# jvmncs/safe-grid-agents

Measured on AMD Instinct MI355X. Metric: env-steps/sec at 1M concurrent BoatRace envs, higher is better.
Workload: dtype int8

## Files before the change

safe-grid-agents_amd/csrc/sgk_api.hip:

```cpp
#include <hip/hip_runtime.h>

#include <algorithm>
#include <cmath>
#include <cstdio>
#include <cstdlib>
#include <cstring>
#include <memory>
#include <utility>

#include "sgk_host_core.h"
#include "sgk_kernels.h"

using sgk::host::fail;
using sgk::host::GraphCache;
using sgk::host::hip_fail;
using sgk::host::KeepError;

namespace {

__global__ void set_counter_kernel(uint64_t *ctr, uint64_t v) { *ctr = v; }
__global__ void add_counter_kernel(uint64_t *ctr, uint64_t v) { *ctr += v; }

}

// ... 174 lines not shown
  *out = nullptr;
  if (n_envs <= 0 || n_envs > ((int64_t)1 << 31) - 512) return fail(SGK_ERR_INVALID, "n_envs out of range");
  const bool host_visible = (layout & SGK_MEM_HOST_VISIBLE) != 0;
  layout &= ~SGK_MEM_HOST_VISIBLE;
  if (layout != SGK_LAYOUT_PITCHED && layout != SGK_LAYOUT_COMPACT) return fail(SGK_ERR_INVALID, "unknown layout");
  if (host_visible && n_envs > 65536) return fail(SGK_ERR_INVALID, "SGK_MEM_HOST_VISIBLE is for small batches (<= 65536 envs)");
  int n_dev = 0;
  hipError_t e = hipGetDeviceCount(&n_dev);
  if (e != hipSuccess || n_dev <= 0)
    return fail(SGK_ERR_NODEVICE, "libsgk has no CPU fallback and found no HIP device%s%s", e != hipSuccess ? ": " : "",
                e != hipSuccess ? hipGetErrorString(e) : "");
  if (device < 0 || device >= n_dev) return fail(SGK_ERR_INVALID, "device ordinal out of range");
  sgk_env *h = sgk::host::host_new<sgk_env>();
  sgk::Shard &s = h->sh;
  if (sgk_build_rules(env_id, &s.rules_host) != 0) {
    delete h;
    return fail(SGK_ERR_INVALID, "unknown env_id");
  }
  s.env_id = env_id;
  s.device = device;
  s.n = n_envs;
  s.seed = seed;
  s.env_base = env_index_base;
  s.n_cells = s.rules_host.n_cells;
  s.n_states = s.rules_host.n_states;
  const int pitched = ((s.n_cells + 15) / 16) * 16;
  s.layout = layout;
  s.pitch = (s.layout == SGK_LAYOUT_COMPACT) ? s.n_cells : pitched;
  const char *ng = getenv("SGK_NO_GRAPH");
  h->use_graph = !(ng && ng[0] == '1');

#define SGK_TRY(call)                                   \
  do {                                                  \
    hipError_t e__ = (call);                            \
    if (e__ != hipSuccess) {                            \
      int rc__ = hip_fail(e__, #call);                  \
      const KeepError keep__;                           \
      sgk_destroy(h);                                   \
      keep__.restore();                                 \
      return rc__;                                      \
    }                                                   \
  } while (0)

  SGK_TRY(hipSetDevice(device));
  hipDeviceProp_t prop;
  SGK_TRY(hipGetDeviceProperties(&prop, device));
  s.n_cus = prop.multiProcessorCount > 0 ? prop.multiProcessorCount : 256;
  s.max_grid = s.n_cus * 6;
  if (const char *mg = getenv("SGK_MAX_GRID")) {
    int v = atoi(mg);
    if (v >= 64) s.max_grid = v;
  }
  s.stream_grid = s.n_cus * 16;
  if (const char *nt = getenv("SGK_RING_NT")) s.ring_nt_mode = nt[0] == '0' ? 0 : (nt[0] == '1' ? 1 : -1);
  if (const char *sg = getenv("SGK_STREAM_GRID")) {
    int v = atoi(sg);
    if (v >= 64) s.stream_grid = v;
  }
  s.rollout_grid = s.n_cus * 12;
  SGK_TRY(pooled_stream(device, &h->own_stream));
  h->stream = h->own_stream;
  const int64_t n_pad = ((s.n + 255) / 256) * 256;
  const int64_t n_wg = n_pad / 256;
  SGK_TRY(hipMalloc((void **)&s.rules_dev, sgk::SGK_RULES_DEV_BYTES));
  h->host_visible = host_visible;
  if (host_visible) {
    SGK_TRY(hipHostMalloc((void **)&s.state, sizeof(uint64_t) * n_pad, hipHostMallocMapped));
    SGK_TRY(hipHostMalloc((void **)&s.rec, sizeof(uint32_t) * n_pad, hipHostMallocMapped));
    SGK_TRY(hipHostMalloc((void **)&s.boards, (size_t)s.pitch * n_pad, hipHostMallocMapped));
    SGK_TRY(hipHostMalloc((void **)&h->hv_actions, (size_t)n_pad, hipHostMallocMapped));
    const char *srv = getenv("SGK_STEP_SERVER");
    if (n_envs <= 64 && !(srv && srv[0] == '0')) {
      SGK_TRY(hipHostMalloc((void **)&h->srv.mb, sizeof(sgk::SgkMailbox), hipHostMallocMapped));
      memset((void *)h->srv.mb, 0, sizeof(sgk::SgkMailbox));
    }
  } else {
    SGK_TRY(hipMalloc(&s.state, sizeof(uint64_t) * n_pad));
    SGK_TRY(hipMalloc(&s.rec, sizeof(uint32_t) * n_pad));
    SGK_TRY(hipMalloc(&s.boards, (size_t)s.pitch * n_pad));
  }
  if (host_visible) {
    SGK_TRY(hipHostMalloc((void **)&s.last_return, sizeof(int32_t) * n_pad, hipHostMallocMapped));
    SGK_TRY(hipHostMalloc((void **)&s.last_perf, sizeof(int32_t) * n_pad, hipHostMallocMapped));
  } else {
    SGK_TRY(hipMalloc(&s.last_return, sizeof(int32_t) * n_pad));
    SGK_TRY(hipMalloc(&s.last_perf, sizeof(int32_t) * n_pad));
  }
  SGK_TRY(hipMalloc(&s.n_episodes, sizeof(int32_t) * n_pad));
  SGK_TRY(hipMalloc(&s.n_resets, sizeof(int32_t) * n_pad));
  if (env_id == SGK_FRIEND_FOE) SGK_TRY(hipMalloc(&s.aux, sizeof(double) * SGK_AUX_DOUBLES * n_pad));
  SGK_TRY(hipMalloc(&s.metrics, sizeof(int64_t) * SGK_METRICS_LEN));
  SGK_TRY(hipMalloc(&s.metric_slab, sizeof(int64_t) * SGK_METRICS_LEN * SGK_METRIC_SLOTS));
  SGK_TRY(hipMalloc(&s.wg_count, sizeof(int32_t) * n_wg));
  SGK_TRY(hipMalloc(&s.wg_offset, sizeof(int64_t) * n_wg));
  SGK_TRY(hipMalloc(&s.finished_total, sizeof(int64_t)));
  SGK_TRY(hipMalloc(&h->t_dev, sizeof(uint64_t)));
  SGK_TRY(hipHostMalloc((void **)&h->metrics_pinned, sizeof(long long) * SGK_METRICS_LEN, hipHostMallocMapped));
  {
    static_assert(sgk::SGK_RULES_DEV_BYTES <= 8192, "staged on the stack");
    uint8_t image[sgk::SGK_RULES_DEV_BYTES];
    memset(image, 0, sizeof(image));
    memcpy(image, &s.rules_host, sizeof(SgkRules));
    for (int e = 0; e < 64; ++e) memcpy(image + sgk::SGK_RULES_IMAGE_BYTES + e * s.n_cells, s.rules_host.templ, (size_t)s.n_cells);
    SGK_TRY(hipMemcpyAsync(s.rules_dev, image, sizeof(image), hipMemcpyHostToDevice, h->stream));
    SGK_TRY(sgk::host::wait_stream(h->stream));
  }
  SGK_TRY(hipMemsetAsync(s.rec, 0, sizeof(uint32_t) * n_pad, h->stream));
// ... 1263 lines not shown
```

safe-grid-agents_amd/csrc/sgk_host_core.h:

```cpp
#pragma once
#include <hip/hip_runtime.h>
#include <stdarg.h>
#include <stdint.h>
#include <stdio.h>
#include <string.h>

#include <atomic>
#include <map>
#include <memory>
#include <mutex>
#include <new>
#include <utility>
#include <vector>

#include "../../include/sgk.h"
#include "sgk_mailbox.h"

namespace sgk {
namespace host {

constexpr size_t ERROR_BYTES = 640;
inline char *error_buffer() {
  static thread_local char buf[ERROR_BYTES] = "";
  return buf;
}
__attribute__((format(printf, 2, 3))) inline int fail(int code, const char *fmt, ...) {
  char tmp[ERROR_BYTES];
  va_list ap;
  va_start(ap, fmt);
  vsnprintf(tmp, sizeof(tmp), fmt, ap);
  va_end(ap);
  memcpy(error_buffer(), tmp, sizeof(tmp));
  return code;
}
inline int hip_fail(hipError_t e, const char *what) { return fail(SGK_ERR_HIP, "%s: %s", what, hipGetErrorString(e)); }
struct KeepError {
  char saved[ERROR_BYTES];
  KeepError() { memcpy(saved, error_buffer(), ERROR_BYTES); }
  void restore() const { memcpy(error_buffer(), saved, ERROR_BYTES); }
};

#define SGK_HIP(call)                                               \
  do {                                                              \
    hipError_t e__ = (call);                                        \
    if (e__ != hipSuccess) return ::sgk::host::hip_fail(e__, #call); \
  } while (0)

#define SGK_CATCH_STATUS                                                                                        \
  catch (const std::bad_alloc &) { return ::sgk::host::fail(SGK_ERR_NOMEM, "out of host memory"); }           \
  catch (const std::exception &e__) { return ::sgk::host::fail(SGK_ERR_INTERNAL, "internal error: %s", e__.what()); } \
  catch (...) { return ::sgk::host::fail(SGK_ERR_INTERNAL, "internal error (unknown exception)"); }
#define SGK_CATCH_VALUE(v) \
  catch (...) { return (v); }

inline std::atomic<int> &alloc_countdown() {
  static std::atomic<int> c{0};
  return c;
}
inline void alloc_gate() {
  std::atomic<int> &c = alloc_countdown();
  if (c.load(std::memory_order_relaxed) > 0 && c.fetch_sub(1, std::memory_order_relaxed) == 1) throw std::bad_alloc();
}
template <class T>
struct HostAlloc {
  using value_type = T;
  HostAlloc() = default;
  template <class U>
  HostAlloc(const HostAlloc<U> &) {}
  T *allocate(size_t n) {
    alloc_gate();
    return std::allocator<T>().allocate(n);
  }
  void deallocate(T *p, size_t n) { std::allocator<T>().deallocate(p, n); }
  template <class U>
  bool operator==(const HostAlloc<U> &) const { return true; }
  template <class U>
  bool operator!=(const HostAlloc<U> &) const { return false; }
};
template <class T>
using Vec = std::vector<T, HostAlloc<T>>;
template <class K, class V>
using Map = std::map<K, V, std::less<K>, HostAlloc<std::pair<const K, V>>>;
template <class T>
T *host_new() {
  alloc_gate();
  return new T();
}
// ... 379 lines not shown
```

safe-grid-agents_amd/csrc/sgk_kernels.h:

```cpp
#pragma once
#include <hip/hip_runtime.h>
#include <stdint.h>

#include "../../include/sgk.h"
#include "sgk_mailbox.h"
#include "sgk_rules.h"

#define SGK_METRIC_SLOTS 2048

namespace sgk {

constexpr int SGK_RULES_IMAGE_BYTES = 2048;
constexpr int SGK_RULES_DEV_BYTES = SGK_RULES_IMAGE_BYTES + 64 * SGK_CELLS;

struct Shard {
  int env_id = 0, layout = 0, device = 0;
  int n_cells = 0, pitch = 0, n_states = 0;
  int n_cus = 256, max_grid = 2048, stream_grid = 2048, rollout_grid = 2048;
  int ring_nt_mode = -1;
  int64_t n = 0;
  uint64_t seed = 0, env_base = 0, lockstep_t = 0;
  SgkRules rules_host;
  SgkRules *rules_dev = nullptr;
  uint64_t *state = nullptr;
  uint32_t *rec = nullptr;
  int8_t *boards = nullptr;
  int32_t *last_return = nullptr;
  int32_t *last_perf = nullptr;
  int32_t *n_episodes = nullptr;
  int32_t *n_resets = nullptr;
  double *aux = nullptr;
  int64_t *metrics = nullptr;
  int64_t *metric_slab = nullptr;
  int32_t *wg_count = nullptr;
  int64_t *wg_offset = nullptr;
  int64_t *finished_total = nullptr;
};

struct TabqShard {
  double *table = nullptr;
  uint64_t *tags = nullptr;
  double *row_cache = nullptr;
  uint32_t *keys = nullptr;
  int32_t hash_cap = 0;
  int32_t *hash_overflow = nullptr;
  int32_t n_states = 0;
  double lr = 0, discount = 0, eps0 = 0;
  int64_t anneal = 0;
  int64_t t_agent = 0;
  const long long *t_ptr = nullptr;
};

hipError_t launch_step(const Shard &sh, const uint8_t *actions, uint32_t flags, hipStream_t st);
hipError_t launch_env_server(const Shard &sh, const uint8_t *actions, SgkMailbox *mb, uint32_t last, hipStream_t st);
hipError_t launch_rollout_random(const Shard &sh, int32_t n_steps, uint32_t flags, hipStream_t st);
hipError_t launch_rollout_stream(const Shard &sh, int32_t n_steps, uint32_t flags, int8_t *boards_ring, uint32_t *recs_ring,
                                 int32_t ring, int32_t slice0, hipStream_t st);
hipError_t launch_reset(const Shard &sh, const uint8_t *mask, int mode, hipStream_t st);
hipError_t launch_ring_probe(const Shard &sh, int8_t *boards_ring, uint32_t *recs_ring, int32_t ring, uint32_t flags, hipStream_t st);
hipError_t launch_metrics_init(const Shard &sh, hipStream_t st);
hipError_t launch_aux_init(const Shard &sh, hipStream_t st);
hipError_t launch_metrics_reduce(const Shard &sh, hipStream_t st, long long *out_host = nullptr);
hipError_t launch_obs_f32(const Shard &sh, float *dst, hipStream_t st);
struct PolicyWeights {
  const float *w1t, *b1, *w2, *b2, *w3t, *b3;
  int n_hidden;
};
hipError_t launch_policy_act(const Shard &sh, int mode, const PolicyWeights &w, uint8_t *actions, float *scores, double eps,
                             uint64_t draw, const double *eps_dev, const uint64_t *draw_dev, hipStream_t st);
hipError_t launch_policy_rollout(const Shard &sh, int mode, const PolicyWeights &w, double eps, uint64_t draw0, int32_t n_steps,
                                 uint32_t flags, int8_t *states_out, uint8_t *actions_out, uint32_t *recs_out, hipStream_t st);
hipError_t launch_eps_greedy(const Shard &sh, int mode, const float *scores, uint8_t *actions, double eps, uint64_t draw,
// ... 109 lines not shown
```

safe-grid-agents_amd/csrc/sgk_step.hip:

```cpp
#include <type_traits>

#include "sgk_device.h"
#include "sgk_step_store.h"

namespace sgk {

constexpr int STREAM_MIN_WAVES = 4;
#define SGK_TILE_DECLARE(ENV, NC, ON)                                                 \
  __shared__ __attribute__((aligned(16))) uint8_t tile_images[WG / 64][64 * (NC)];    \
  WaveTileLds<ENV, NC> W;                                                             \
  W.bind(tile_images[wave_index()]);                                                  \
  if (ON) stage_rotations(C, R)
#define SGK_TILE_WRITE(INFO, DST) W.write(C, R, (INFO), (DST))

__global__ __launch_bounds__(1024) void metrics_reduce_kernel(const long long *__restrict__ slab, long long *__restrict__ out,
                                                              long long *__restrict__ out_host) {
  __shared__ long long part[1024];
  const int col = threadIdx.x & 15, lane_slot = threadIdx.x >> 4;
  const bool is_max = col >= SGK_M_MAX_RETURN && col <= SGK_M_MAX_MARGIN_POS;
  long long acc = is_max ? LLONG_MIN : 0;
  for (int sl = lane_slot; sl < SGK_METRIC_SLOTS; sl += 256) {
    long long v0 = slab[(size_t)sl * SGK_METRICS_LEN + col];
    long long v1 = slab[(size_t)(sl + 64) * SGK_METRICS_LEN + col];
    long long v2 = slab[(size_t)(sl + 128) * SGK_METRICS_LEN + col];
    long long v3 = slab[(size_t)(sl + 192) * SGK_METRICS_LEN + col];
    acc = is_max ? max(max(acc, v0), max(max(v1, v2), v3)) : acc + ((v0 + v1) + (v2 + v3));
  }
  part[threadIdx.x] = acc;
  __syncthreads();
  for (int half = 32; half >= 1; half >>= 1) {
    if (lane_slot < half) {
      long long o = part[(lane_slot + half) * 16 + col];
      part[threadIdx.x] = is_max ? max(part[threadIdx.x], o) : part[threadIdx.x] + o;
    }
    __syncthreads();
  }
  if (threadIdx.x < 16) {
    out[threadIdx.x] = part[threadIdx.x];
    if (out_host) out_host[threadIdx.x] = part[threadIdx.x];
  }
}

__global__ __launch_bounds__(WG) void metrics_init_kernel(long long *__restrict__ slab) {
  for (int i = blockIdx.x * WG + threadIdx.x; i < SGK_METRIC_SLOTS * SGK_METRICS_LEN; i += gridDim.x * WG) {
    int col = i & 15;
    slab[i] = (col >= SGK_M_MAX_RETURN && col <= SGK_M_MAX_MARGIN_POS) ? LLONG_MIN : 0;
  }
}

constexpr int64_t STEP_SMALL_MAX_ENVS = 65536;

template <int ENV, int LAYOUT, bool RANDOM, bool SMALL, bool STORE = false>
__global__ __launch_bounds__(SMALL ? 64 : WG) void step_kernel(StepArgs a, StepStore st) {
  constexpr int WGT = SMALL ? 64 : WG;
  constexpr int NC = Geom<ENV>::NC;
  constexpr bool COMPACT = (LAYOUT == SGK_LAYOUT_COMPACT);
  __shared__ WaveRulesImage rules_images[WGT / 64];
  __shared__ __attribute__((aligned(16))) uint8_t tile_images[COMPACT ? WGT / 64 : 1][COMPACT ? 64 * NC : 16];
  __shared__ int episode_words[WGT / 64][16];
  const int lane = threadIdx.x & 63, wave = wave_index();
  const int64_t n_wt = (a.n + 63) / 64;
  const int64_t wt0 = (int64_t)blockIdx.x * (WGT / 64) + wave, wstride = (int64_t)gridDim.x * (WGT / 64);
  const bool boards_on = !(a.flags & SGK_F_NO_BOARDS);
  keep_in_sgprs(a.rec, a.boards, a.last_return, a.last_perf);
  keep_in_sgprs(a.n_episodes, a.n_resets, a.metrics, a.aux);
  keep_in_sgprs(a.seed, a.env_base, a.t, a.flags);
// ... 124 lines not shown
    if (req == SGK_SERVER_STOP) break;
    idle_since = 0;
    const uint32_t flags = hi & 0xffu;
    int action = (int)((hi >> 8) & 3u);
    if (a.n > 1) {
      __builtin_amdgcn_fence(__ATOMIC_ACQUIRE, "");
      if (valid) action = (int)(__hip_atomic_load(&a.actions[env], __ATOMIC_RELAXED, __HIP_MEMORY_SCOPE_SYSTEM) & 3u);
    }
    if (flags & SGK_SRV_RESET) {
      if (valid) {
        const int epi = s.epi + 1;
        bump_reset_count<ENV>(a.n_resets, env);
        s = initial_state(R);
        s.epi = epi;
        begin_episode<ENV>(R, s, a.seed, a.env_base + (uint64_t)env, aux_of<ENV>(a.aux, env));
        a.state[env] = pack_state(s);
      }
    } else {
      StepArgs b = a;
      b.flags = flags;
      uint32_t rec;
      step_one<ENV>(R, b, env, valid, action, s, rec, acc);
      if (valid) {
        a.state[env] = pack_state(s);
        a.rec[env] = rec;
      }
    }
    if (!(flags & SGK_F_NO_BOARDS)) {
      if (COMPACT) {
        W.draw_all(C, R, sprite_info<ENV>(R, s));
        W.flush_prefix(a.boards, (int)a.n * NC);
      } else if (valid) {
        write_board_pitched<ENV, Geom<ENV>::PITCH>(R, a.boards, env, s);
      }
    }
    __builtin_amdgcn_fence(__ATOMIC_RELEASE, "");
    asm volatile("s_waitcnt vmcnt(0)" ::: "memory");
    if (lane == 0) __hip_atomic_store(&mb->done, req, __ATOMIC_RELAXED, __HIP_MEMORY_SCOPE_SYSTEM);
    last = req;
  }
  acc_flush(acc, a.metrics);
  __builtin_amdgcn_fence(__ATOMIC_RELEASE, "");
  asm volatile("s_waitcnt vmcnt(0)" ::: "memory");
  if (lane == 0) __hip_atomic_store(&mb->exited, last + 1u, __ATOMIC_RELAXED, __HIP_MEMORY_SCOPE_SYSTEM);
}

hipError_t launch_env_server(const Shard &sh, const uint8_t *actions, SgkMailbox *mb, uint32_t last, hipStream_t st) {
  (void)hipGetLastError();
  StepArgs a = make_step_args(sh, actions, 0);
  SGK_DISPATCH_ENV_LAYOUT(sh.env_id, sh.layout, env_server_kernel<E, L><<<dim3(1), dim3(64), 0, st>>>(a, mb, last));
  return hipGetLastError();
}

struct StreamOut {
  int8_t *boards;
  uint32_t *recs;
  int32_t ring, slice0;
  int32_t tiles_ok;
  int32_t tile_major;
  int32_t ring_nt;
};

template <int ENV, int LAYOUT, bool STREAM>
__global__ __launch_bounds__(WG, STREAM ? STREAM_MIN_WAVES : 1) void rollout_random_kernel(StepArgs a, int32_t n_steps, StreamOut o) {
  constexpr int NC = Geom<ENV>::NC;
  constexpr bool COMPACT = (LAYOUT == SGK_LAYOUT_COMPACT);
  __shared__ SgkRules R;
  __shared__ CompactLds<NC> C;
  uint64_t first_word = 0;
  {
    const int64_t env0 = ((int64_t)blockIdx.x * (WG / 64) + (threadIdx.x >> 6)) * 64 + (threadIdx.x & 63);
    if (STREAM && env0 < a.n) first_word = a.state[env0];
  }
  stage_rules(R, a.rules);
  SGK_TILE_DECLARE(ENV, NC, (COMPACT || STREAM));
  const int lane = threadIdx.x & 63, wave = STREAM ? wave_index() : (int)(threadIdx.x >> 6);
  const bool boards_on = !(a.flags & SGK_F_NO_BOARDS);
  const int64_t n_wt = (a.n + 63) / 64;
  EpisodeAcc acc;
  acc_init(acc);
  for (int64_t wt = (int64_t)blockIdx.x * (WG / 64) + wave; wt < n_wt; wt += (int64_t)gridDim.x * (WG / 64)) {
    const int64_t env = wt * 64 + lane;
    const bool valid = env < a.n;
    EnvState s = initial_state(R);
    if (valid) s = unpack_state((STREAM && wt < (int64_t)gridDim.x * (WG / 64)) ? first_word : a.state[env]);
    load_episode_index<ENV>(s, a.n_resets, env, valid);
    const uint64_t ge = a.env_base + (uint64_t)env;
    AuxRegs ax;
    ax.init();
    if (HasAux<ENV>::value && valid) ax.load(a.aux + env * SGK_AUX_DOUBLES);
    uint32_t x[4] = {0, 0, 0, 0};
    uint32_t rec = 0;
    uint32_t w = 0;
    int last_obs = 0, last_hid = 0, last_done = 0, last_action = 0;
    const bool auto_reset = (a.flags & SGK_F_AUTO_RESET) != 0;
    const bool whole_tile = wt * 64 + 64 <= a.n;
    int32_t slice = o.slice0;
    uint32_t drawn = sprite_info<ENV>(R, s);
    if (STREAM && boards_on) W.draw_all(C, R, drawn);
    if (STREAM) {
    const bool tm = o.boards && o.tile_major;
    const bool tiles = o.boards ? (tm || (o.tiles_ok && whole_tile)) : COMPACT;
    const bool flush_nt = o.boards && o.ring_nt;
    uint32_t *recs_p = !o.recs ? a.rec + env
                               : (o.tile_major ? o.recs + (wt * (int64_t)o.ring + slice) * 64 + lane : o.recs + (int64_t)slice * a.n + env);
    const int64_t rec_stride = !o.recs ? 0 : (o.tile_major ? 64 : a.n);
    int8_t *dense = !o.boards ? a.boards
                              : (tm ? o.boards + ((wt * (int64_t)o.ring + slice) - wt) * 64 * NC : o.boards + (int64_t)slice * a.n * NC);
    const int64_t brd_stride = !o.boards ? 0 : (tm ? (int64_t)64 * NC : a.n * (int64_t)NC);
    const int64_t rec_wrap = rec_stride * (o.ring - 1), brd_wrap = brd_stride * (o.ring - 1);
    uint32_t left = 0;
#pragma nounroll
    for (int32_t k = 0; k < n_steps; ++k) {
      if (left == 0) {
        const uint64_t t = a.t + (uint64_t)k;
        const uint32_t tl = (uint32_t)t;
        if (k == 0 || (tl & 63u) == 0)
          philox4x32_10((uint32_t)ge, (uint32_t)(ge >> 32), (uint32_t)(t >> 6), 0u, (uint32_t)a.seed, (uint32_t)(a.seed >> 32), x);
        const uint32_t j = (tl >> 4) & 3u;
        w = (j == 0 ? x[0] : (j == 1 ? x[1] : (j == 2 ? x[2] : x[3]))) >> (2 * (tl & 15u));
        left = 16 - (tl & 15u);
      }
      --left;
      int action = (int)(w & 3u);
      w >>= 2;
      const bool live = valid && !s.over;
      if (live) action = env_actual_action<ENV>(R, s, a.seed, ge, action);
      last_action = action;
      last_obs = 0;
      last_hid = 0;
      last_done = valid ? 1 : 0;
      if (live) {
        int r_obs, r_hid, term;
        if (HasAux<ENV>::value) transition_with<ENV>(R, s, action, r_obs, r_hid, term, ax);
        else transition<ENV>(R, s, action, r_obs, r_hid, term);
        s.frame += 1;
        s.ret += r_obs;
        s.hid += r_hid;
        last_obs = r_obs;
        last_hid = r_hid;
        last_done = 0;
        if (term || s.frame >= R.max_iterations) {
          last_done = 1;
          acc_add(acc, true, s.ret, s.hid);
          int64_t env_here = env;
          asm volatile("" : "+v"(env_here));
          a.last_return[env_here] = s.ret;
          a.last_perf[env_here] = s.hid;
          bump_episode_count(a.n_episodes, env_here);
          if (auto_reset) {
            const int epi = s.epi + 1;
            s = initial_state(R);
            s.epi = epi;
            if (HasAux<ENV>::value) begin_episode_with<ENV>(R, s, a.seed, ge, ax);
            else begin_episode<ENV>(R, s, a.seed, ge);
          } else {
            s.over = 1;
          }
        }
      }
      const uint32_t rk = pack_rec(last_obs, last_hid, last_done, last_action);
      if (valid) *recs_p = rk;
      if (boards_on) {
        const uint32_t now = sprite_info<ENV>(R, s);
        W.update(R, drawn, now);
        drawn = now;
        if (tiles) {
          if (flush_nt) W.template flush<RING_STORE_AUX>(dense + wt * 64 * NC);
          else W.flush(dense + wt * 64 * NC);
        }
        else if (o.boards) { if (valid) write_row_bytes<ENV, NC>(R, dense + env * NC, s); }
        else if (valid) write_board_pitched<ENV, Geom<ENV>::PITCH>(R, a.boards, env, s);
      }
      if (++slice == o.ring) {
        slice = 0;
        recs_p -= rec_wrap;
        dense -= brd_wrap;
      } else {
        recs_p += rec_stride;
        dense += brd_stride;
      }
    }
    if (boards_on && o.boards && tiles && COMPACT && n_steps > 0) W.flush(a.boards + wt * 64 * NC);
    } else {
      auto one_step = [&](int action, auto check) {
        constexpr bool CHECK = decltype(check)::value;
        const bool live = CHECK ? (valid && !s.over) : true;
        if (live) action = env_actual_action<ENV>(R, s, a.seed, ge, action);
        last_action = action;
        if (live) {
          int r_obs, r_hid, term;
          if (HasAux<ENV>::value) transition_with<ENV>(R, s, action, r_obs, r_hid, term, ax);
          else transition<ENV>(R, s, action, r_obs, r_hid, term);
          s.frame += 1;
          s.ret += r_obs;
          s.hid += r_hid;
          last_obs = r_obs;
          last_hid = r_hid;
          last_done = 0;
          if (term || s.frame >= R.max_iterations) {
            last_done = 1;
            acc_add(acc, true, s.ret, s.hid);
            a.last_return[env] = s.ret;
            a.last_perf[env] = s.hid;
            bump_episode_count(a.n_episodes, env);
            if (auto_reset) {
              const int epi = s.epi + 1;
              s = initial_state(R);
              s.epi = epi;
              if (HasAux<ENV>::value) begin_episode_with<ENV>(R, s, a.seed, ge, ax);
              else begin_episode<ENV>(R, s, a.seed, ge);
            } else {
              s.over = 1;
            }
          }
        } else {
          last_obs = 0;
          last_hid = 0;
          last_done = valid ? 1 : 0;
        }
      };
      const bool lean = auto_reset && whole_tile && (__ballot(s.over != 0) == 0ull);
      uint64_t t = a.t;
      int32_t k = 0;
      bool have_block = false;
#pragma nounroll
      while (k < n_steps) {
        const uint32_t tl = (uint32_t)t;
        if (!have_block || (tl & 63u) == 0u) {
          philox4x32_10((uint32_t)ge, (uint32_t)(ge >> 32), (uint32_t)(t >> 6), 0u, (uint32_t)a.seed, (uint32_t)(a.seed >> 32), x);
          have_block = true;
        }
        const uint32_t j = (tl >> 4) & 3u;
        w = (j == 0 ? x[0] : (j == 1 ? x[1] : (j == 2 ? x[2] : x[3]))) >> (2 * (tl & 15u));
        const int32_t m = min((int32_t)(16u - (tl & 15u)), n_steps - k);
        if (lean) {
#pragma nounroll
          for (int32_t i = 0; i < m; ++i) {
            one_step((int)(w & 3u), std::false_type{});
            w >>= 2;
          }
        } else {
#pragma nounroll
          for (int32_t i = 0; i < m; ++i) {
            one_step((int)(w & 3u), std::true_type{});
            w >>= 2;
          }
        }
        k += m;
        t += (uint64_t)m;
      }
    }
    rec = pack_rec(last_obs, last_hid, last_done, last_action);
    if (valid) {
      a.state[env] = pack_state(s);
      if (!STREAM || o.recs) a.rec[env] = rec;
      if (HasEnvDraws<ENV>::value) a.n_resets[env] = s.epi;
      if (HasAux<ENV>::value && ax.dirty) ax.store(a.aux + env * SGK_AUX_DOUBLES);
    }
    if (!STREAM && boards_on) {
      if (COMPACT) SGK_TILE_WRITE(sprite_info<ENV>(R, s), a.boards + wt * 64 * NC);
      else if (valid) write_board_pitched<ENV, Geom<ENV>::PITCH>(R, a.boards, env, s);
    }
  }
  acc_flush(acc, a.metrics);
}

template <int ENV, int LAYOUT, bool STORE = false>
__global__ __launch_bounds__(WG) void reset_kernel(const SgkRules *rules, uint64_t *state, int8_t *boards,
                                                   const uint8_t *mask, int mode_flags, int64_t n, uint64_t seed, uint64_t env_base,
                                                   int32_t *__restrict__ n_resets, const double *__restrict__ aux, StepStore st) {
  reset_body<ENV, LAYOUT, STORE>(rules, state, boards, mask, mode_flags, n, seed, env_base, n_resets, aux, st, (int)blockIdx.x, (int)gridDim.x);
}

__global__ __launch_bounds__(WG) void obs_f32_kernel(const int8_t *__restrict__ boards, float *__restrict__ dst, int64_t n,
                                                     int nc, int pitch) {
  const int q_per_env = (nc + 3) / 4;
  const int64_t total = n * q_per_env;
  for (int64_t i = (int64_t)blockIdx.x * blockDim.x + threadIdx.x; i < total; i += (int64_t)gridDim.x * blockDim.x) {
    int64_t env = i / q_per_env;
    int q = (int)(i - env * q_per_env);
    const int8_t *src = boards + env * pitch + q * 4;
    float *out = dst + env * nc + q * 4;
    if (q * 4 + 4 <= nc && ((nc & 3) == 0) && ((pitch & 3) == 0)) {
      uint32_t w = *reinterpret_cast<const uint32_t *>(src);
      float4 f = make_float4((float)(int8_t)(w & 0xff), (float)(int8_t)((w >> 8) & 0xff),
                             (float)(int8_t)((w >> 16) & 0xff), (float)(int8_t)(w >> 24));
      *reinterpret_cast<float4 *>(out) = f;
    } else {
      for (int k = 0; k < 4 && q * 4 + k < nc; ++k) out[k] = (float)src[k];
    }
  }
}

__global__ __launch_bounds__(WG) void render_rgb_kernel(const SgkRules *__restrict__ rules, const int8_t *__restrict__ boards,
                                                        uint8_t *__restrict__ dst, int64_t n, int nc, int pitch) {
  __shared__ uint8_t pal[8][4];
  if (threadIdx.x < 32) (&pal[0][0])[threadIdx.x] = (&rules->palette[0][0])[threadIdx.x];
  __syncthreads();
  const bool hwc = rules->render_hwc != 0;
  const int64_t total = n * nc;
  for (int64_t i = (int64_t)blockIdx.x * blockDim.x + threadIdx.x; i < total; i += (int64_t)gridDim.x * blockDim.x) {
    int64_t env = i / nc;
    int c = (int)(i - env * nc);
    int v = boards[env * pitch + c] & 7;
    uint8_t *o = dst + env * 3 * nc + (hwc ? 3 * c : c);
    const int plane = hwc ? 1 : nc;
    o[0] = pal[v][0];
    o[plane] = pal[v][1];
    o[2 * plane] = pal[v][2];
  }
}

__global__ __launch_bounds__(WG) void dense_boards_kernel(const int8_t *__restrict__ boards, int8_t *__restrict__ dst,
// ... 72 lines not shown

hipError_t launch_step_counter(const Shard &sh, const uint64_t *t_dev, uint64_t t_off, uint32_t flags, hipStream_t st) {
  (void)hipGetLastError();
  StepArgs a = make_step_args(sh, nullptr, flags);
  a.t = t_off;
  a.t_ptr = t_dev;
  if (sh.n <= STEP_SMALL_MAX_ENVS) {
    SGK_DISPATCH_ENV_LAYOUT(sh.env_id, sh.layout, step_kernel<E, L, true, true><<<dim3((unsigned)((sh.n + 63) / 64)), dim3(64), 0, st>>>(a, StepStore{}));
  } else {
    int grid = grid_for((sh.n + WG - 1) / WG, sh.max_grid);
    SGK_DISPATCH_ENV_LAYOUT(sh.env_id, sh.layout, step_kernel<E, L, true, false><<<dim3(grid), dim3(WG), 0, st>>>(a, StepStore{}));
  }
  return hipGetLastError();
}

hipError_t launch_step(const Shard &sh, const uint8_t *actions, uint32_t flags, hipStream_t st) {
  (void)hipGetLastError();
  StepArgs a = make_step_args(sh, actions, flags);
  const bool small = sh.n <= STEP_SMALL_MAX_ENVS;
  const dim3 grid(small ? (unsigned)((sh.n + 63) / 64) : (unsigned)grid_for((sh.n + WG - 1) / WG, sh.max_grid)), block(small ? 64 : WG);
  if (actions) {
    if (small) SGK_DISPATCH_ENV_LAYOUT(sh.env_id, sh.layout, step_kernel<E, L, false, true><<<grid, block, 0, st>>>(a, StepStore{}));
    else SGK_DISPATCH_ENV_LAYOUT(sh.env_id, sh.layout, step_kernel<E, L, false, false><<<grid, block, 0, st>>>(a, StepStore{}));
  } else {
    if (small) SGK_DISPATCH_ENV_LAYOUT(sh.env_id, sh.layout, step_kernel<E, L, true, true><<<grid, block, 0, st>>>(a, StepStore{}));
    else SGK_DISPATCH_ENV_LAYOUT(sh.env_id, sh.layout, step_kernel<E, L, true, false><<<grid, block, 0, st>>>(a, StepStore{}));
  }
  return hipGetLastError();
}


hipError_t launch_step_store(const Shard &sh, const uint8_t *actions, uint32_t flags, int cheat, int64_t slice, const long long *slice_dev,
                             int32_t ring, int8_t *successors, uint8_t *r_actions, int8_t *r_rewards, uint8_t *r_terminals, hipStream_t st) {
  (void)hipGetLastError();
  StepArgs a = make_step_args(sh, actions, flags);
  const StepStore so = make_store(sh, successors, r_actions, r_rewards, r_terminals, slice, slice_dev, ring, cheat);
  const bool small = sh.n <= STEP_SMALL_MAX_ENVS;
  const dim3 grid(small ? (unsigned)((sh.n + 63) / 64) : (unsigned)grid_for((sh.n + WG - 1) / WG, sh.max_grid)), block(small ? 64 : WG);
  if (small) SGK_DISPATCH_ENV_LAYOUT(sh.env_id, sh.layout, step_kernel<E, L, false, true, true><<<grid, block, 0, st>>>(a, so));
  else SGK_DISPATCH_ENV_LAYOUT(sh.env_id, sh.layout, step_kernel<E, L, false, false, true><<<grid, block, 0, st>>>(a, so));
  return hipGetLastError();
}

hipError_t launch_rollout_random(const Shard &sh, int32_t n_steps, uint32_t flags, hipStream_t st) {
  (void)hipGetLastError();
  StepArgs a = make_step_args(sh, nullptr, flags);
  int grid = grid_for((sh.n + WG - 1) / WG, sh.rollout_grid);
  StreamOut o{nullptr, nullptr, 1, 0, 0, 0, 0};
  SGK_DISPATCH_ENV_LAYOUT(sh.env_id, sh.layout,
                          rollout_random_kernel<E, L, false><<<dim3(grid), dim3(WG), 0, st>>>(a, n_steps, o));
  return hipGetLastError();
}

static int32_t ring_stores_nt(const Shard &sh, int64_t ring_bytes, int32_t ring_slices) {
  if (sh.ring_nt_mode >= 0) return sh.ring_nt_mode;
  return ring_slices >= 48 && ring_bytes > (256ll << 20);
}

hipError_t launch_rollout_stream(const Shard &sh, int32_t n_steps, uint32_t flags, int8_t *boards_ring, uint32_t *recs_ring,
                                 int32_t ring, int32_t slice0, hipStream_t st) {
  (void)hipGetLastError();
  StepArgs a = make_step_args(sh, nullptr, flags);
  int grid = grid_for((sh.n + WG - 1) / WG, sh.stream_grid);
  StreamOut o{boards_ring, recs_ring, ring < 1 ? 1 : ring, slice0, (int32_t)(((sh.n * sh.n_cells) % 16) == 0 && ((uintptr_t)boards_ring % 16) == 0),
              (int32_t)((flags & SGK_F_RING_TILE_MAJOR) != 0),
              ring_stores_nt(sh, (int64_t)(ring < 1 ? 1 : ring) * sh.n * (sh.n_cells + 4), ring)};
  SGK_DISPATCH_ENV_LAYOUT(sh.env_id, sh.layout,
                          rollout_random_kernel<E, L, true><<<dim3(grid), dim3(WG), 0, st>>>(a, n_steps, o));
  hipError_t e = hipGetLastError();
  if (e != hipSuccess) return e;
  const bool in_kernel = sh.layout == SGK_LAYOUT_COMPACT && (o.tile_major || (o.tiles_ok && sh.n % 64 == 0));
  if (boards_ring && !(flags & SGK_F_NO_BOARDS) && !in_kernel) return launch_reset(sh, nullptr, 2, st);
  return hipSuccess;
}

template <int NC>
__global__ __launch_bounds__(WG) void ring_probe_kernel(int8_t *boards, uint32_t *recs, int64_t n, int32_t ring, int32_t tile_major,
                                                       int32_t nt) {
  constexpr int BYTES = 64 * NC, CHUNKS = 4 * NC, ITS = (CHUNKS + 63) / 64;
  const int lane = threadIdx.x & 63, wave = wave_index();
  const int64_t n_wt = n / 64;
  const sgk_u32x4 zero = {0u, 0u, 0u, 0u};
  for (int64_t wt = (int64_t)blockIdx.x * (WG / 64) + wave; wt < n_wt; wt += (int64_t)gridDim.x * (WG / 64)) {
    for (int32_t s = 0; s < ring; ++s) {
      if (boards) {
        int8_t *dst = tile_major ? boards + (wt * (int64_t)ring + s) * BYTES : boards + ((int64_t)s * n + wt * 64) * NC;
        const __amdgpu_buffer_rsrc_t rsrc = __builtin_amdgcn_make_buffer_rsrc((void *)dst, 0, BYTES, 0x00020000);
#pragma unroll
        for (int it = 0; it < ITS; ++it) {
          if (nt) __builtin_amdgcn_raw_buffer_store_b128(zero, rsrc, (lane + 64 * it) * 16, 0, RING_STORE_AUX);
          else __builtin_amdgcn_raw_buffer_store_b128(zero, rsrc, (lane + 64 * it) * 16, 0, BOARD_STORE_AUX);
        }
      }
      if (recs) {
        uint32_t *r = tile_major ? recs + (wt * (int64_t)ring + s) * 64 + lane : recs + (int64_t)s * n + wt * 64 + lane;
        *r = 0u;
      }
    }
  }
}

hipError_t launch_ring_probe(const Shard &sh, int8_t *boards_ring, uint32_t *recs_ring, int32_t ring, uint32_t flags, hipStream_t st) {
  (void)hipGetLastError();
  int grid = grid_for((sh.n + WG - 1) / WG, sh.stream_grid);
  const int32_t tm = (flags & SGK_F_RING_TILE_MAJOR) != 0;
  const int32_t nt = ring_stores_nt(sh, (int64_t)ring * sh.n * (sh.n_cells + 4), ring);
  SGK_DISPATCH_ENV(sh.env_id, (ring_probe_kernel<Geom<E>::NC><<<dim3(grid), dim3(WG), 0, st>>>(boards_ring, recs_ring, sh.n, ring, tm, nt)));
  return hipGetLastError();
}

hipError_t launch_reset(const Shard &sh, const uint8_t *mask, int mode, hipStream_t st) {
  (void)hipGetLastError();
  int grid = grid_for((sh.n + WG - 1) / WG, sh.max_grid);
  SGK_DISPATCH_ENV_LAYOUT(sh.env_id, sh.layout,
                          reset_kernel<E, L><<<dim3(grid), dim3(WG), 0, st>>>(sh.rules_dev, sh.state,
                                              sh.boards, mask, mode, sh.n, sh.seed, sh.env_base, sh.n_resets, sh.aux, StepStore{}));
  return hipGetLastError();
}

hipError_t launch_reset_done_store(const Shard &sh, uint32_t flags, int64_t slice, const long long *slice_dev, int32_t ring, int8_t *states,
                                   hipStream_t st) {
  (void)hipGetLastError();
  int grid = grid_for((sh.n + WG - 1) / WG, sh.max_grid);
  const StepStore so = make_store(sh, states, nullptr, nullptr, nullptr, slice, slice_dev, ring, 0);
  const int mode = 1 | ((flags & SGK_F_NO_BOARDS) ? 4 : 0);
  SGK_DISPATCH_ENV_LAYOUT(sh.env_id, sh.layout,
                          reset_kernel<E, L, true><<<dim3(grid), dim3(WG), 0, st>>>(sh.rules_dev, sh.state,
                                              sh.boards, nullptr, mode, sh.n, sh.seed, sh.env_base, sh.n_resets, sh.aux, so));
  return hipGetLastError();
}

__global__ __launch_bounds__(WG) void fill_f64_kernel(double *__restrict__ dst, int64_t count, double value) {
  for (int64_t i = (int64_t)blockIdx.x * WG + threadIdx.x; i < count; i += (int64_t)gridDim.x * WG) dst[i] = value;
}

hipError_t launch_aux_init(const Shard &sh, hipStream_t st) {
  (void)hipGetLastError();
  if (!sh.aux) return hipSuccess;
  const int64_t count = sh.n * SGK_AUX_DOUBLES;
  fill_f64_kernel<<<dim3(grid_for((count + WG - 1) / WG, sh.max_grid)), dim3(WG), 0, st>>>(sh.aux, count, 0.5);
  return hipGetLastError();
}

hipError_t launch_metrics_init(const Shard &sh, hipStream_t st) {
  (void)hipGetLastError();
  metrics_init_kernel<<<dim3(32), dim3(WG), 0, st>>>((long long *)sh.metric_slab);
  return hipGetLastError();
}

hipError_t launch_metrics_reduce(const Shard &sh, hipStream_t st, long long *out_host) {
  (void)hipGetLastError();
  metrics_reduce_kernel<<<dim3(1), dim3(1024), 0, st>>>((const long long *)sh.metric_slab, (long long *)sh.metrics, out_host);
  return hipGetLastError();
}

hipError_t launch_obs_f32(const Shard &sh, float *dst, hipStream_t st) {
  (void)hipGetLastError();
  int64_t total = sh.n * ((sh.n_cells + 3) / 4);
  int grid = grid_for((total + WG - 1) / WG, sh.max_grid * 4);
// ... 32 lines not shown
```

Baseline: 221.9 billion.

## Add 1024-thread cluster path for streamed ring rollouts with double-buffered LDS flush

Adds a clustered variant of the streaming rollout kernel. It uses 1024-thread workgroups, one per 1024 consecutive envs, and double-buffers per-wave board tiles in LDS. After a block barrier, each step's boards for the whole cluster are written as one contiguous run of 128-bit buffer stores instead of separate per-wave tiles. The path is enabled by default for compact layouts at 256K envs or more, or set by an environment knob, and the ring probe kernel gets a matching variant. The aim is larger, more coalesced streaming writes to the ring. The cost is a __syncthreads per step, double the LDS for tiles, one resident wave-tile loop per block instead of a grid-stride loop, and possibly lower occupancy.

```diff
diff --git a/safe-grid-agents_amd/csrc/sgk_api.hip b/safe-grid-agents_amd/csrc/sgk_api.hip
--- a/safe-grid-agents_amd/csrc/sgk_api.hip
+++ b/safe-grid-agents_amd/csrc/sgk_api.hip
@@ -250,7 +250,8 @@
     if (v >= 64) s.max_grid = v;
   }
   s.stream_grid = s.n_cus * 16;
-  if (const char *nt = getenv("SGK_RING_NT")) s.ring_nt_mode = nt[0] == '0' ? 0 : (nt[0] == '1' ? 1 : -1);
+  s.ring_nt_mode = sgk::host::knob_0_1(getenv("SGK_RING_NT"));
+  s.ring_cluster_mode = sgk::host::knob_0_1(getenv("SGK_RING_CLUSTER"));
   if (const char *sg = getenv("SGK_STREAM_GRID")) {
     int v = atoi(sg);
     if (v >= 64) s.stream_grid = v;
diff --git a/safe-grid-agents_amd/csrc/sgk_host_core.h b/safe-grid-agents_amd/csrc/sgk_host_core.h
--- a/safe-grid-agents_amd/csrc/sgk_host_core.h
+++ b/safe-grid-agents_amd/csrc/sgk_host_core.h
@@ -33,6 +33,8 @@
   memcpy(error_buffer(), tmp, sizeof(tmp));
   return code;
 }
+inline int knob_0_1(const char *value) { return !value ? -1 : (value[0] == '0' ? 0 : (value[0] == '1' ? 1 : -1)); }
+
 inline int hip_fail(hipError_t e, const char *what) { return fail(SGK_ERR_HIP, "%s: %s", what, hipGetErrorString(e)); }
 struct KeepError {
   char saved[ERROR_BYTES];
diff --git a/safe-grid-agents_amd/csrc/sgk_kernels.h b/safe-grid-agents_amd/csrc/sgk_kernels.h
--- a/safe-grid-agents_amd/csrc/sgk_kernels.h
+++ b/safe-grid-agents_amd/csrc/sgk_kernels.h
@@ -18,6 +18,7 @@
   int n_cells = 0, pitch = 0, n_states = 0;
   int n_cus = 256, max_grid = 2048, stream_grid = 2048, rollout_grid = 2048;
   int ring_nt_mode = -1;
+  int ring_cluster_mode = -1;
   int64_t n = 0;
   uint64_t seed = 0, env_base = 0, lockstep_t = 0;
   SgkRules rules_host;
diff --git a/safe-grid-agents_amd/csrc/sgk_step.hip b/safe-grid-agents_amd/csrc/sgk_step.hip
--- a/safe-grid-agents_amd/csrc/sgk_step.hip
+++ b/safe-grid-agents_amd/csrc/sgk_step.hip
@@ -6,12 +6,7 @@
 namespace sgk {
 
 constexpr int STREAM_MIN_WAVES = 4;
-#define SGK_TILE_DECLARE(ENV, NC, ON)                                                 \
-  __shared__ __attribute__((aligned(16))) uint8_t tile_images[WG / 64][64 * (NC)];    \
-  WaveTileLds<ENV, NC> W;                                                             \
-  W.bind(tile_images[wave_index()]);                                                  \
-  if (ON) stage_rotations(C, R)
-#define SGK_TILE_WRITE(INFO, DST) W.write(C, R, (INFO), (DST))
+constexpr int CLUSTER_WG = 1024;
 
 __global__ __launch_bounds__(1024) void metrics_reduce_kernel(const long long *__restrict__ slab, long long *__restrict__ out,
                                                               long long *__restrict__ out_host) {
@@ -242,6 +237,26 @@
   return hipGetLastError();
 }
 
+template <int NC, int AUX>
+__device__ __forceinline__ void cluster_flush(const uint8_t *images, int8_t *run, int wave, int lane) {
+  constexpr int ITS = (NC + 15) / 16;
+  const __amdgpu_buffer_rsrc_t rsrc = __builtin_amdgcn_make_buffer_rsrc((void *)run, 0, NC * 1024, 0x00020000);
+  uint4 v[ITS];
+#pragma unroll
+  for (int it = 0; it < ITS; ++it) {
+    const int i = wave + 16 * it;
+    if (16 * it + 15 < NC || i < NC) v[it] = *reinterpret_cast<const uint4 *>(images + (i * 64 + lane) * 16);
+  }
+#pragma unroll
+  for (int it = 0; it < ITS; ++it) {
+    const int i = wave + 16 * it;
+    if (16 * it + 15 < NC || i < NC) {
+      sgk_u32x4 v4 = {v[it].x, v[it].y, v[it].z, v[it].w};
+      __builtin_amdgcn_raw_buffer_store_b128(v4, rsrc, (i * 64 + lane) * 16, 0, AUX);
+    }
+  }
+}
+
 struct StreamOut {
   int8_t *boards;
   uint32_t *recs;
@@ -251,29 +266,33 @@
   int32_t ring_nt;
 };
 
-template <int ENV, int LAYOUT, bool STREAM>
-__global__ __launch_bounds__(WG, STREAM ? STREAM_MIN_WAVES : 1) void rollout_random_kernel(StepArgs a, int32_t n_steps, StreamOut o) {
+template <int ENV, int LAYOUT, bool STREAM, bool CLUSTER = false>
+__global__ __launch_bounds__(CLUSTER ? CLUSTER_WG : WG, (STREAM && !CLUSTER) ? STREAM_MIN_WAVES : 1) void rollout_random_kernel(StepArgs a, int32_t n_steps, StreamOut o) {
   constexpr int NC = Geom<ENV>::NC;
   constexpr bool COMPACT = (LAYOUT == SGK_LAYOUT_COMPACT);
+  constexpr int WAVES = (CLUSTER ? CLUSTER_WG : WG) / 64;
   __shared__ SgkRules R;
   __shared__ CompactLds<NC> C;
   uint64_t first_word = 0;
   {
-    const int64_t env0 = ((int64_t)blockIdx.x * (WG / 64) + (threadIdx.x >> 6)) * 64 + (threadIdx.x & 63);
+    const int64_t env0 = ((int64_t)blockIdx.x * WAVES + (threadIdx.x >> 6)) * 64 + (threadIdx.x & 63);
     if (STREAM && env0 < a.n) first_word = a.state[env0];
   }
   stage_rules(R, a.rules);
-  SGK_TILE_DECLARE(ENV, NC, (COMPACT || STREAM));
+  __shared__ __attribute__((aligned(16))) uint8_t tile_images[CLUSTER ? 2 : 1][WAVES][64 * NC];
+  WaveTileLds<ENV, NC> W;
+  W.bind(tile_images[0][wave_index()]);
+  if (COMPACT || STREAM) stage_rotations(C, R);
   const int lane = threadIdx.x & 63, wave = STREAM ? wave_index() : (int)(threadIdx.x >> 6);
   const bool boards_on = !(a.flags & SGK_F_NO_BOARDS);
   const int64_t n_wt = (a.n + 63) / 64;
   EpisodeAcc acc;
   acc_init(acc);
-  for (int64_t wt = (int64_t)blockIdx.x * (WG / 64) + wave; wt < n_wt; wt += (int64_t)gridDim.x * (WG / 64)) {
+  for (int64_t wt = (int64_t)blockIdx.x * WAVES + wave; wt < n_wt; wt += (int64_t)gridDim.x * WAVES) {
     const int64_t env = wt * 64 + lane;
     const bool valid = env < a.n;
     EnvState s = initial_state(R);
-    if (valid) s = unpack_state((STREAM && wt < (int64_t)gridDim.x * (WG / 64)) ? first_word : a.state[env]);
+    if (valid) s = unpack_state((STREAM && wt < (int64_t)gridDim.x * WAVES) ? first_word : a.state[env]);
     load_episode_index<ENV>(s, a.n_resets, env, valid);
     const uint64_t ge = a.env_base + (uint64_t)env;
     AuxRegs ax;
@@ -288,6 +307,14 @@
     int32_t slice = o.slice0;
     uint32_t drawn = sprite_info<ENV>(R, s);
     if (STREAM && boards_on) W.draw_all(C, R, drawn);
+    const bool cluster = CLUSTER && ((int64_t)blockIdx.x + 1) * CLUSTER_WG <= a.n;
+    uint32_t drawn_other = drawn;
+    int set = 0;
+    if (cluster) {
+      W.bind(tile_images[CLUSTER ? 1 : 0][wave]);
+      W.draw_all(C, R, drawn);
+      W.bind(tile_images[0][wave]);
+    }
     if (STREAM) {
     const bool tm = o.boards && o.tile_major;
     const bool tiles = o.boards ? (tm || (o.tiles_ok && whole_tile)) : COMPACT;
@@ -350,12 +377,22 @@
         }
       }
       const uint32_t rk = pack_rec(last_obs, last_hid, last_done, last_action);
-      if (valid) *recs_p = rk;
+      if (!cluster && valid) *recs_p = rk;
       if (boards_on) {
         const uint32_t now = sprite_info<ENV>(R, s);
         W.update(R, drawn, now);
         drawn = now;
-        if (tiles) {
+        if (cluster) {
+          __syncthreads();
+          *recs_p = rk;
+          int8_t *run = dense + (int64_t)blockIdx.x * (WAVES * 64 * NC);
+          if (flush_nt) cluster_flush<NC, RING_STORE_AUX>(&tile_images[set][0][0], run, wave, lane);
+          else cluster_flush<NC, BOARD_STORE_AUX>(&tile_images[set][0][0], run, wave, lane);
+          set ^= 1;
+          W.bind(tile_images[CLUSTER ? set : 0][wave]);
+          drawn = drawn_other;
+          drawn_other = now;
+        } else if (tiles) {
           if (flush_nt) W.template flush<RING_STORE_AUX>(dense + wt * 64 * NC);
           else W.flush(dense + wt * 64 * NC);
         }
@@ -371,6 +408,7 @@
         dense += brd_stride;
       }
     }
+    if (cluster) W.bind(tile_images[CLUSTER ? set ^ 1 : 0][wave]);
     if (boards_on && o.boards && tiles && COMPACT && n_steps > 0) W.flush(a.boards + wt * 64 * NC);
     } else {
       auto one_step = [&](int action, auto check) {
@@ -449,7 +487,7 @@
       if (HasAux<ENV>::value && ax.dirty) ax.store(a.aux + env * SGK_AUX_DOUBLES);
     }
     if (!STREAM && boards_on) {
-      if (COMPACT) SGK_TILE_WRITE(sprite_info<ENV>(R, s), a.boards + wt * 64 * NC);
+      if (COMPACT) W.write(C, R, sprite_info<ENV>(R, s), a.boards + wt * 64 * NC);
       else if (valid) write_board_pitched<ENV, Geom<ENV>::PITCH>(R, a.boards, env, s);
     }
   }
@@ -628,9 +666,18 @@
   return hipGetLastError();
 }
 
+constexpr int64_t RING_CLUSTER_MIN_ENVS = 262144;
 static int32_t ring_stores_nt(const Shard &sh, int64_t ring_bytes, int32_t ring_slices) {
   if (sh.ring_nt_mode >= 0) return sh.ring_nt_mode;
   return ring_slices >= 48 && ring_bytes > (256ll << 20);
+}
+
+static bool ring_cluster(const Shard &sh, uint32_t flags, const int8_t *boards_ring, const uint32_t *recs_ring, int32_t tiles_ok) {
+  const bool can = sh.layout == SGK_LAYOUT_COMPACT && boards_ring && recs_ring && tiles_ok && sh.n >= CLUSTER_WG &&
+                   !(flags & (SGK_F_NO_BOARDS | SGK_F_RING_TILE_MAJOR));
+  if (!can) return false;
+  if (sh.ring_cluster_mode >= 0) return sh.ring_cluster_mode != 0;
+  return sh.n >= RING_CLUSTER_MIN_ENVS;
 }
 
 hipError_t launch_rollout_stream(const Shard &sh, int32_t n_steps, uint32_t flags, int8_t *boards_ring, uint32_t *recs_ring,
@@ -641,8 +688,13 @@
   StreamOut o{boards_ring, recs_ring, ring < 1 ? 1 : ring, slice0, (int32_t)(((sh.n * sh.n_cells) % 16) == 0 && ((uintptr_t)boards_ring % 16) == 0),
               (int32_t)((flags & SGK_F_RING_TILE_MAJOR) != 0),
               ring_stores_nt(sh, (int64_t)(ring < 1 ? 1 : ring) * sh.n * (sh.n_cells + 4), ring)};
-  SGK_DISPATCH_ENV_LAYOUT(sh.env_id, sh.layout,
-                          rollout_random_kernel<E, L, true><<<dim3(grid), dim3(WG), 0, st>>>(a, n_steps, o));
+  if (ring_cluster(sh, flags, boards_ring, recs_ring, o.tiles_ok)) {
+    const int64_t groups = ((sh.n + 63) / 64 + CLUSTER_WG / 64 - 1) / (CLUSTER_WG / 64);
+    SGK_DISPATCH_ENV(sh.env_id, (rollout_random_kernel<E, SGK_LAYOUT_COMPACT, true, true><<<dim3((unsigned)groups), dim3(CLUSTER_WG), 0, st>>>(a, n_steps, o)));
+  } else {
+    SGK_DISPATCH_ENV_LAYOUT(sh.env_id, sh.layout,
+                            rollout_random_kernel<E, L, true><<<dim3(grid), dim3(WG), 0, st>>>(a, n_steps, o));
+  }
   hipError_t e = hipGetLastError();
   if (e != hipSuccess) return e;
   const bool in_kernel = sh.layout == SGK_LAYOUT_COMPACT && (o.tile_major || (o.tiles_ok && sh.n % 64 == 0));
@@ -676,11 +728,50 @@
   }
 }
 
+template <int NC>
+__global__ __launch_bounds__(CLUSTER_WG) void ring_probe_cluster_kernel(int8_t *boards, uint32_t *recs, int64_t n, int32_t ring, int32_t nt) {
+  constexpr int ITS = (NC + 15) / 16, TILE_ITS = (4 * NC + 63) / 64;
+  const int lane = threadIdx.x & 63, wave = wave_index();
+  const int64_t wt = (int64_t)blockIdx.x * (CLUSTER_WG / 64) + wave;
+  const bool cluster = ((int64_t)blockIdx.x + 1) * CLUSTER_WG <= n;
+  const sgk_u32x4 zero = {0u, 0u, 0u, 0u};
+  if (!cluster && wt >= n / 64) return;
+  for (int32_t s = 0; s < ring; ++s) {
+    if (cluster) __syncthreads();
+    recs[(int64_t)s * n + wt * 64 + lane] = 0u;
+    if (cluster) {
+      const __amdgpu_buffer_rsrc_t rsrc =
+          __builtin_amdgcn_make_buffer_rsrc((void *)(boards + ((int64_t)s * n + (int64_t)blockIdx.x * CLUSTER_WG) * NC), 0, NC * 1024, 0x00020000);
+#pragma unroll
+      for (int it = 0; it < ITS; ++it) {
+        const int i = wave + 16 * it;
+        if (16 * it + 15 < NC || i < NC) {
+          if (nt) __builtin_amdgcn_raw_buffer_store_b128(zero, rsrc, (i * 64 + lane) * 16, 0, RING_STORE_AUX);
+          else __builtin_amdgcn_raw_buffer_store_b128(zero, rsrc, (i * 64 + lane) * 16, 0, BOARD_STORE_AUX);
+        }
+      }
+    } else {
+      const __amdgpu_buffer_rsrc_t rsrc = __builtin_amdgcn_make_buffer_rsrc((void *)(boards + ((int64_t)s * n + wt * 64) * NC), 0, 64 * NC, 0x00020000);
+#pragma unroll
+      for (int it = 0; it < TILE_ITS; ++it) {
+        if (nt) __builtin_amdgcn_raw_buffer_store_b128(zero, rsrc, (lane + 64 * it) * 16, 0, RING_STORE_AUX);
+        else __builtin_amdgcn_raw_buffer_store_b128(zero, rsrc, (lane + 64 * it) * 16, 0, BOARD_STORE_AUX);
+      }
+    }
+  }
+}
+
 hipError_t launch_ring_probe(const Shard &sh, int8_t *boards_ring, uint32_t *recs_ring, int32_t ring, uint32_t flags, hipStream_t st) {
   (void)hipGetLastError();
   int grid = grid_for((sh.n + WG - 1) / WG, sh.stream_grid);
   const int32_t tm = (flags & SGK_F_RING_TILE_MAJOR) != 0;
   const int32_t nt = ring_stores_nt(sh, (int64_t)ring * sh.n * (sh.n_cells + 4), ring);
+  const int32_t tiles_ok = ((sh.n * sh.n_cells) % 16) == 0 && ((uintptr_t)boards_ring % 16) == 0;
+  if (ring_cluster(sh, flags, boards_ring, recs_ring, tiles_ok)) {
+    const int64_t groups = (sh.n / 64 + CLUSTER_WG / 64 - 1) / (CLUSTER_WG / 64);
+    SGK_DISPATCH_ENV(sh.env_id, (ring_probe_cluster_kernel<Geom<E>::NC><<<dim3((unsigned)groups), dim3(CLUSTER_WG), 0, st>>>(boards_ring, recs_ring, sh.n, ring, nt)));
+    return hipGetLastError();
+  }
   SGK_DISPATCH_ENV(sh.env_id, (ring_probe_kernel<Geom<E>::NC><<<dim3(grid), dim3(WG), 0, st>>>(boards_ring, recs_ring, sh.n, ring, tm, nt)));
   return hipGetLastError();
 }
```

After: 217.2 billion. 0.979x the previous value.
